# hvasbath/beat

Hardware: AMD Instinct MI355X
Metric: SMC chain-steps/s (FFI seismic gfstacking 400 patches x 64 targets x 4096 samples) (higher is better)
Workload: dtype f64; 1 GPU; BASELINE configs[2]: FFI seismic gfstacking, 400 patches x 64 targets x 4096 samples, library (64,400,3,25,4096) f64 = 62.9 GB in HBM, nearest_neighbor, covariance scalar; population SURVEY 8(d): nucleation U over the 20x20 fault, time 0; chains_per_gpu=512, global_chains=512, parallelism=chains sharded over 1 GPU(s), library replicated

## Files before the change

### beat_amd/csrc/ctx.hpp

```cpp
#pragma once
#include <hip/hip_runtime.h>

#include <cstdarg>
#include <cstdint>
#include <cstdio>
#include <cstring>
#include <map>
#include <memory>
#include <string>
#include <vector>

#include "../../include/beat_amd.h"

struct beatamd_ctx;

namespace beatamd {

void set_error(const char *fmt, ...);

#define BA_HIP(expr)                                                                         \
    do {                                                                                     \
        hipError_t e_ = (expr);                                                              \
        if (e_ != hipSuccess) {                                                              \
            beatamd::set_error("%s:%d: %s -> %s", __FILE__, __LINE__, #expr,                 \
// ... 178 lines not shown
    mutable DevMem<double> pole_coef;
    mutable int64_t pole_chains = 0;
};

struct GeomSources {
    int nsrc = 0;
    DevMem<int32_t> kind;
    DevMem<int64_t> poff;
    DevMem<double> pfix;
    DevMem<double> east, north, los;
    int64_t Nobs = 0;
    double nu = 0.25;
};

struct FfiModel {
    beatamd_ffi_layout layout;
    int32_t nsub = 0;
    std::vector<int32_t> ndip, nstrike, patch_off;
    std::vector<double> patch_size;
    int64_t P = 0;
    DevMem<int32_t> d_ndip, d_nstrike, d_patch_off;
    DevMem<double> d_patch_size;
    std::vector<Wavemap> wavemaps;
    bool has_geo = false;
    Geodetic geo;
    bool geo_is_geometry = false;
    GeomSources geom;
    int32_t lap = -1;
    int64_t nllk() const;
    bool obs_quads_valid = false;
    std::vector<double> obs_quads;
    DevMem<double> d_obs_quads;
    int32_t lsq_var = -1, lsq_zero_var = -1;
    bool lsq_blocks_valid = false;
    DevMem<double> lsq_GG, lsq_LtL;
};

struct HyperModel {
    int64_t nterm = 0, nh = 0;
    DevMem<double> M, slog;
    DevMem<int32_t> kind, hp_index;
    int32_t ngroups = 0, group_end[8] = {0, 0, 0, 0, 0, 0, 0, 0};
};

constexpr int KNOB_UNSET = -2147483647;
#define BEATAMD_GF_KNOBS(X) \
    X(gf_kernel, "BEATAMD_GF_KERNEL") X(gs_cg, "BEATAMD_GS_CG") X(gs_ws, "BEATAMD_GS_WS") X(gs_dma, "BEATAMD_GS_DMA") X(gs_nt, "BEATAMD_GS_NT") \
    X(ws_map, "BEATAMD_WS_MAP") X(gs_pair, "BEATAMD_GS_PAIR") X(gs_nthint, "BEATAMD_GS_NTHINT") X(gs_order, "BEATAMD_GS_ORDER") \
    X(gs_fit, "BEATAMD_GS_FIT") X(gs_win, "BEATAMD_GS_WIN") X(gf_tinv, "BEATAMD_GF_TINV") X(gs_tune, "BEATAMD_GS_TUNE") \
    X(gf_order, "BEATAMD_GF_ORDER") X(gf_cgroup, "BEATAMD_GF_CGROUP") X(gs_ml, "BEATAMD_GS_ML") X(gc_global, "BEATAMD_GC_GLOBAL") \
    X(gc_sort, "BEATAMD_GC_SORT") X(gc_keys, "BEATAMD_GC_KEYS") X(gc_bands, "BEATAMD_GC_BANDS") X(gr_cap, "BEATAMD_GR_CAP") \
    X(gr_pass_alloc, "BEATAMD_GR_PASS_ALLOC") X(gr_var, "BEATAMD_GR_VAR") X(sweep_v1, "BEATAMD_SWEEP_V1") X(qf_band, "BEATAMD_QF_BAND") \
    X(qf_fuse, "BEATAMD_QF_FUSE") X(gf_split, "BEATAMD_GF_SPLIT") X(gm_wave, "BEATAMD_GM_WAVE") X(skip_parked, "BEATAMD_SKIP_PARKED") \
    X(td_strip, "BEATAMD_TD_STRIP")
struct GfKnobs {
#define X(member, env) int member = KNOB_UNSET;
    BEATAMD_GF_KNOBS(X)
#undef X
    void read_env();
    static int get(int v, int dflt) { return v == KNOB_UNSET ? dflt : v; }
    static bool is(int v, int x) { return v != KNOB_UNSET && v == x; }
    static bool set(int v) { return v != KNOB_UNSET; }
};

struct KTimer {
    double total_ms = 0;
    int64_t n = 0;
    std::vector<std::pair<hipEvent_t, hipEvent_t>> pending;
};

}

struct beatamd_ctx {
    int device = 0;
    hipStream_t stream = nullptr, own_stream = nullptr;
    bool timing = false;
    std::map<std::string, beatamd::KTimer> timers;
    std::vector<hipEvent_t> event_pool;
    int *d_status = nullptr;
    std::vector<beatamd::DevBuf> scratch_bufs;
    std::vector<std::unique_ptr<beatamd::SeisStore>> seislibs;
    std::vector<std::unique_ptr<beatamd::GeoLib>> geolibs;
    std::vector<std::unique_ptr<beatamd::GeoEnsemble>> geoens;
    std::vector<std::unique_ptr<beatamd::WeightSet>> wsets;
    std::vector<std::unique_ptr<beatamd::Laplacian>> laps;
    std::vector<std::unique_ptr<beatamd::FfiModel>> models;
    std::vector<std::unique_ptr<beatamd::HyperModel>> hypers;
    int num_cu = 256;
    char last_gf_kernel[96] = "";
    int64_t gs_ngtp = 0, gs_N = 0;
    double gs_trep = 1;
    int gs_nvar = 1;
    bool gs_has_passes = false;
    char gf_plan[384] = "";
    char gf_tune_log[512] = "";
    uint32_t *h_umax = nullptr;
    hipEvent_t umax_event = nullptr;
    bool umax_pending = false;
    int umax_hist = -1, umax_hist_cg = 0;
    std::map<std::vector<int64_t>, std::pair<int, int>> gs_tuned;
    int gs_cg = 0;
    beatamd::GfKnobs knobs;
    bool knobs_live = false;
    uint32_t *step_dev = nullptr;
    std::map<int64_t, beatamd::DevMem<double>> twiddles;

    int get_scratch(int slot, size_t bytes, void **out);
// ... 69 lines not shown
```

### beat_amd/csrc/gfshared.hip

```cpp
#include "kernels.hpp"
#include "misfit.hpp"

namespace beatamd {

constexpr int GS_NT_MAX = 64;
constexpr int GS_NTHINT_DEFAULT = 1;
constexpr int GS_WS_DEFAULT = 1;

struct GroupTabArgs {
    int nrow, nvar, CG;
    int64_t C, T, P, DS;
    const uint32_t *rowoff;
    const double *fac;
    ChainVec slips[4];
    int ucap, ustride;
    uint32_t *urows;
    uint32_t *uent;
    int nissue;
    int windowed;
    int depth;
    uint32_t *ucount;
    uint32_t *umax;
    uint16_t *slot;
    double *w;
// ... 97 lines not shown
                int cost = (tid < 32 && wcnt < a.depth)
                    ? ((__popc(wmask & mm) << 12) | (wcnt << 6) | tid) : 0x7fffffff;
#pragma unroll
                for (int off = 32; off > 0; off >>= 1) cost = min(cost, __shfl_xor(cost, off, 64));
                const int w = cost & 63;
                if (tid == w) {
                    slt[ridx] = (uint32_t)(w + 32 * wcnt);
                    wmask |= mm;
                    wcnt++;
                }
            }
        }
        __syncthreads();
        for (int i = tid; i < total; i += CG) flags[lst[i]] = slt[i];
        __syncthreads();
    }
    {
        const uint32_t last = total > 0 ? a.urows[gtp * a.ustride + total - 1] : (uint32_t)row0;
        for (int i = total + tid; i < a.ustride; i += CG) a.urows[gtp * a.ustride + i] = last;
        const int nw = a.nissue, kstr = a.ustride / nw;
        for (int i = tid; i < a.ustride; i += CG) {
            const uint32_t r = (i < total) ? a.urows[gtp * a.ustride + i] : last;
            uint32_t *e = a.uent + ((gtp * nw + (i % nw)) * kstr + (i / nw)) * 2;
            e[0] = r;
            e[1] = (i < total) ? flags[r - (uint32_t)row0] : 0u;
        }
    }
    for (int k = 0; k < a.nrow; k++)
        a.slot[(gtp * a.nrow + k) * CG + tid] = live ? (uint16_t)flags[v[k]] : (uint16_t)0;
    for (int iv = 0; iv < a.nvar; iv++) {
        double s = 0.0;
        if (live) s = a.slips[iv].base[c * a.slips[iv].stride + a.slips[iv].off + p];
        double *w = a.w + (int64_t)iv * a.w_var_stride;
        if (a.nrow == 1) {
            if (t == 0) w[(g * a.P + p) * CG + tid] = s;
        } else {
            for (int k = 0; k < 4; k++) {
                double f = live ? a.fac[((c * a.T + t) * a.P + p) * 4 + k] : 0.0;
                w[(gtp * 4 + k) * CG + tid] = f * s;
            }
        }
    }
}

struct GsArgs {
    const double *G[4];
    const float *G32[4];
    int f32pair;
    int nvar, nrow;
    int64_t C, T, P, N;
    int CG, ucap, ustride, ntile, nt;
    int dma;
    int ws;
    int nthint;
    int xcd_order;
    int64_t ngroups;
    const int32_t *tslot;
    int64_t Ttab, rows_per_target;
    const uint32_t *guard_umax;
    int guard_mode, guard_fit;
    const uint32_t *nv;
    int64_t vmax;
    const uint32_t *order;
    const uint32_t *urows, *uent, *ucount;
    const uint16_t *slot;
    const double *w;
    int64_t w_var_stride;
    const double *data, *wscalar;
    double *out, *partial;
    const double *band_w;
    double *edges;
};

typedef double v2d __attribute__((ext_vector_type(2)));

template <int OFF>
__device__ __forceinline__ void lds_rd8(v2d (&x)[8], uint32_t addr, int tok)
{
    asm("ds_read_b128 %0, %8 offset:%c10\n\t"
        "ds_read_b128 %1, %8 offset:%c10+16\n\t"
        "ds_read_b128 %2, %8 offset:%c10+32\n\t"
        "ds_read_b128 %3, %8 offset:%c10+48\n\t"
        "ds_read_b128 %4, %8 offset:%c10+64\n\t"
        "ds_read_b128 %5, %8 offset:%c10+80\n\t"
        "ds_read_b128 %6, %8 offset:%c10+96\n\t"
        "ds_read_b128 %7, %8 offset:%c10+112"
        : "=v"(x[0]), "=v"(x[1]), "=v"(x[2]), "=v"(x[3]), "=v"(x[4]), "=v"(x[5]), "=v"(x[6]), "=v"(x[7])
        : "v"(addr), "s"(tok), "n"(OFF));
}

template <int NLEFT>
__device__ __forceinline__ void lds_wait8(v2d (&x)[8])
{
    asm("s_waitcnt lgkmcnt(%c8)"
        : "+v"(x[0]), "+v"(x[1]), "+v"(x[2]), "+v"(x[3]), "+v"(x[4]), "+v"(x[5]), "+v"(x[6]), "+v"(x[7])
        : "n"(NLEFT));
}

template <int OFF>
__device__ __forceinline__ void lds_rd8_b64(double (&x)[8], uint32_t addr, int tok)
{
    asm("ds_read_b64 %0, %8 offset:%c10\n\t"
        "ds_read_b64 %1, %8 offset:%c10+8\n\t"
        "ds_read_b64 %2, %8 offset:%c10+16\n\t"
        "ds_read_b64 %3, %8 offset:%c10+24\n\t"
        "ds_read_b64 %4, %8 offset:%c10+32\n\t"
        "ds_read_b64 %5, %8 offset:%c10+40\n\t"
        "ds_read_b64 %6, %8 offset:%c10+48\n\t"
        "ds_read_b64 %7, %8 offset:%c10+56"
        : "=v"(x[0]), "=v"(x[1]), "=v"(x[2]), "=v"(x[3]), "=v"(x[4]), "=v"(x[5]), "=v"(x[6]), "=v"(x[7])
        : "v"(addr), "s"(tok), "n"(OFF));
}

template <int OFF>
__device__ __forceinline__ void lds_rd8_b32(float (&x)[8], uint32_t addr, int tok)
{
    asm("ds_read_b32 %0, %8 offset:%c10\n\t"
        "ds_read_b32 %1, %8 offset:%c10+4\n\t"
        "ds_read_b32 %2, %8 offset:%c10+8\n\t"
        "ds_read_b32 %3, %8 offset:%c10+12\n\t"
        "ds_read_b32 %4, %8 offset:%c10+16\n\t"
        "ds_read_b32 %5, %8 offset:%c10+20\n\t"
        "ds_read_b32 %6, %8 offset:%c10+24\n\t"
        "ds_read_b32 %7, %8 offset:%c10+28"
        : "=v"(x[0]), "=v"(x[1]), "=v"(x[2]), "=v"(x[3]), "=v"(x[4]), "=v"(x[5]), "=v"(x[6]), "=v"(x[7])
        : "v"(addr), "s"(tok), "n"(OFF));
}

typedef float v2f __attribute__((ext_vector_type(2)));

template <int SCALE, int OFF, typename PAIR>
__device__ __forceinline__ void lds_rd4_pair(PAIR (&x)[4], uint32_t addr, int tok)
{
    if constexpr (SCALE == 1)
        asm("ds_read_b64 %0, %4 offset:%c6\n\t"
            "ds_read_b64 %1, %4 offset:%c6+8\n\t"
            "ds_read_b64 %2, %4 offset:%c6+16\n\t"
            "ds_read_b64 %3, %4 offset:%c6+24"
            : "=v"(x[0]), "=v"(x[1]), "=v"(x[2]), "=v"(x[3])
            : "v"(addr), "s"(tok), "n"(OFF));
    else
        asm("ds_read_b128 %0, %4 offset:%c6\n\t"
            "ds_read_b128 %1, %4 offset:%c6+16\n\t"
            "ds_read_b128 %2, %4 offset:%c6+32\n\t"
            "ds_read_b128 %3, %4 offset:%c6+48"
            : "=v"(x[0]), "=v"(x[1]), "=v"(x[2]), "=v"(x[3])
            : "v"(addr), "s"(tok), "n"(2 * OFF));
}

template <int NLEFT, typename PAIR>
__device__ __forceinline__ void lds_wait4_pair(PAIR (&x)[4])
{
    asm("s_waitcnt lgkmcnt(%c4)" : "+v"(x[0]), "+v"(x[1]), "+v"(x[2]), "+v"(x[3]) : "n"(NLEFT));
}

template <int NLEFT>
__device__ __forceinline__ void lds_wait8_b64(double (&x)[8])
{
    asm("s_waitcnt lgkmcnt(%c8)"
        : "+v"(x[0]), "+v"(x[1]), "+v"(x[2]), "+v"(x[3]), "+v"(x[4]), "+v"(x[5]), "+v"(x[6]), "+v"(x[7])
        : "n"(NLEFT));
}


// ... 449 lines not shown
            for (int gq = 0; gq < NG; gq++) {
                v2f(&cur)[4] = (gq & 1) ? yb : ya;
                if (gq + 1 < NG) lds_wait4_pair<4>(cur); else lds_wait4_pair<0>(cur);
                __builtin_amdgcn_sched_barrier(0);
#pragma unroll
                for (int q = 0; q < 4; q++) {
                    acc[gq * 8 + 2 * q] = fma((double)cur[q].x, w, acc[gq * 8 + 2 * q]);
                    acc[gq * 8 + 2 * q + 1] = fma((double)cur[q].y, w, acc[gq * 8 + 2 * q + 1]);
                }
                __builtin_amdgcn_sched_barrier(0);
                if (gq + 2 < NG) switch (gq + 2) {
                case 2: lds_rd4_pair<1, 64>(cur, xs, s); break;
                case 3: lds_rd4_pair<1, 96>(cur, xs, s); break;
                case 4: lds_rd4_pair<1, 128>(cur, xs, s); break;
                case 5: lds_rd4_pair<1, 160>(cur, xs, s); break;
                case 6: lds_rd4_pair<1, 192>(cur, xs, s); break;
                case 7: lds_rd4_pair<1, 224>(cur, xs, s); break;
                default: break;
                }
                __builtin_amdgcn_sched_barrier(0);
            }
        }
    }
    GS_DMA_FINISH()
}



#define BA_FMA8 \
    "v_fmac_f64 %0, %8, %16\n\tv_fmac_f64 %1, %9, %16\n\tv_fmac_f64 %2, %10, %16\n\tv_fmac_f64 %3, %11, %16\n\t" \
    "v_fmac_f64 %4, %12, %16\n\tv_fmac_f64 %5, %13, %16\n\tv_fmac_f64 %6, %14, %16\n\tv_fmac_f64 %7, %15, %16\n\t"
#define BA_RD8(OFF) \
    "ds_read_b64 %8, %17 offset:" #OFF "\n\tds_read_b64 %9, %17 offset:" #OFF "+8\n\t" \
    "ds_read_b64 %10, %17 offset:" #OFF "+16\n\tds_read_b64 %11, %17 offset:" #OFF "+24\n\t" \
    "ds_read_b64 %12, %17 offset:" #OFF "+32\n\tds_read_b64 %13, %17 offset:" #OFF "+40\n\t" \
    "ds_read_b64 %14, %17 offset:" #OFF "+48\n\tds_read_b64 %15, %17 offset:" #OFF "+56"
#define BA_ACC8(G) \
    "+v"(acc[G * 8]), "+v"(acc[G * 8 + 1]), "+v"(acc[G * 8 + 2]), "+v"(acc[G * 8 + 3]), "+v"(acc[G * 8 + 4]), \
        "+v"(acc[G * 8 + 5]), "+v"(acc[G * 8 + 6]), "+v"(acc[G * 8 + 7])
#define BA_Y8(Y) "+v"(Y[0]), "+v"(Y[1]), "+v"(Y[2]), "+v"(Y[3]), "+v"(Y[4]), "+v"(Y[5]), "+v"(Y[6]), "+v"(Y[7])
#define BA_FMA4A \
    "v_fmac_f64 %0, %8, %16\n\tv_fmac_f64 %1, %9, %16\n\tv_fmac_f64 %2, %10, %16\n\tv_fmac_f64 %3, %11, %16\n\t"
#define BA_FMA4B \
    "v_fmac_f64 %4, %12, %16\n\tv_fmac_f64 %5, %13, %16\n\tv_fmac_f64 %6, %14, %16\n\tv_fmac_f64 %7, %15, %16\n\t"
#define BA_RD4A(OFF) \
    "ds_read_b64 %8, %17 offset:" #OFF "\n\tds_read_b64 %9, %17 offset:" #OFF "+8\n\t" \
    "ds_read_b64 %10, %17 offset:" #OFF "+16\n\tds_read_b64 %11, %17 offset:" #OFF "+24\n\t"
#define BA_RD4B(OFF) \
    "ds_read_b64 %12, %17 offset:" #OFF "+32\n\tds_read_b64 %13, %17 offset:" #OFF "+40\n\t" \
    "ds_read_b64 %14, %17 offset:" #OFF "+48\n\tds_read_b64 %15, %17 offset:" #OFF "+56"
#define BA_GROUP(G, Y, OFFNEXT) \
    asm("s_waitcnt lgkmcnt(12)\n\t" BA_FMA4A BA_RD4A(OFFNEXT) "s_waitcnt lgkmcnt(12)\n\t" BA_FMA4B BA_RD4B(OFFNEXT) \
        : BA_ACC8(G), BA_Y8(Y) : "v"(w), "v"(xs))

template <int NROW, int MODE, int NB, int NTH>
__global__ void __launch_bounds__(768) __attribute__((amdgpu_waves_per_eu(3, 3)))
k_gfstack_ws(GsArgs a)
{
    constexpr int CW = 8, LW = 4;
    constexpr int GS_NT = 64;
    constexpr int GS_PITCH = GS_NT + 1;
    constexpr int KPRE = 16;
    extern __shared__ __attribute__((aligned(16))) double xbuf[];
    constexpr int CG = CW * 64;
    const int tid = threadIdx.x, lane = tid & 63;
    const int wave = __builtin_amdgcn_readfirstlane(tid >> 6);
    GS_BLOCK_DECODE(a, g, t, tile)
    int64_t gt, tbase;
    gs_table_cell(a, g, t, gt, tbase);
    const int64_t N = a.N;
    const int64_t n0 = (int64_t)tile * GS_NT;
    const uint32_t lds0 = (uint32_t)(uintptr_t)(__attribute__((address_space(3))) void *)xbuf;
    const int bufsz = (a.ucap + 1) * GS_PITCH;
    const int P = a.nv ? (int)__builtin_amdgcn_readfirstlane((int)a.nv[gt]) : (int)a.P;
    const int nvar = a.nvar;
    const int nsteps = P * nvar;

    if (wave >= CW) {
        GS_LOADER_PROGRAM(0, 8, double, G_a = a.G[iv] + tbase)
        return;
    }

    static_assert(NROW == 1, "the loader / consumer kernel exists for single-row interpolation");
    const int64_t c = a.order ? (int64_t)a.order[g * CG + tid] : g * CG + tid;
    for (int i = tid; i < NB * GS_PITCH; i += CG) xbuf[(i / GS_PITCH) * bufsz + a.ucap * GS_PITCH + (i % GS_PITCH)] = 0.0;
    __builtin_amdgcn_fence(__ATOMIC_RELEASE, "workgroup");
    double acc[GS_NT];
#pragma unroll
    for (int i = 0; i < GS_NT; i++) acc[i] = 0.0;
    uint32_t sl_n;
    double wl_n;
    const uint32_t voff_s = (uint32_t)tid * 2u;
    const char *const slot_base = reinterpret_cast<const char *>(a.slot + (gt * a.vmax) * CG);
    const char *const w_base = reinterpret_cast<const char *>(a.w + (gt * a.vmax) * CG);
    const uint32_t slot_step = (uint32_t)(CG * 2);
    const uint32_t w_step = (uint32_t)(CG * 8);
    const int64_t w_var_bytes = a.w_var_stride * 8;
    auto tab_slot = [&](int p) { return slot_base + (uint32_t)p * slot_step; };
    auto tab_w = [&](int p, int iv) {
        return w_base + (uint32_t)p * w_step + (nvar == 1 ? (int64_t)0 : (int64_t)iv * w_var_bytes);
    };
    auto fetch_tabs = [&](const char *ps, const char *pw) {
        asm("global_load_ushort %0, %1, %2" : "=v"(sl_n) : "v"(voff_s), "s"(ps));
        uint32_t voff_w;
        asm("v_lshlrev_b32 %1, 2, %2\n\t"
            "global_load_dwordx2 %0, %1, %3" : "=v"(wl_n), "=&v"(voff_w) : "v"(voff_s), "s"(pw));
    };
    auto row_address = [&](uint32_t base) {
        uint32_t x;
        asm("s_waitcnt vmcnt(0)\n\t"
            "v_lshl_add_u32 %0, %1, 6, %1\n\t"
            "v_lshl_add_u32 %0, %0, 3, %2" : "=&v"(x) : "v"(sl_n), "s"(base), "v"(wl_n));
        return x;
    };
    auto landed_weight = [&](uint32_t after) {
        double x;
        asm("v_mov_b64 %0, %1" : "=v"(x) : "v"(wl_n), "v"(after));
        return x;
    };
    static_assert(GS_PITCH == 65, "row_address multiplies by 65");
    constexpr int NG8 = GS_NT / 8;
    static_assert(NG8 == 8, "the read schedule below is written for 64-sample tiles");
    double ya[8], yb[8];
    int p1 = 0, iv1 = 0;
    gs_advance(p1, iv1, P, nvar);
    int gbuf = 0;
    const int ring = NB * bufsz;
    double w;
    uint32_t xs;
    if (__ballot(c < a.C) == 0) {
        for (int s = 0; s <= nsteps; s++) __builtin_amdgcn_s_barrier();
    } else {
    fetch_tabs(tab_slot(0), tab_w(0, 0));
    xs = row_address(lds0);
    w = landed_weight(xs);
    __builtin_amdgcn_sched_barrier(0);
    __builtin_amdgcn_s_barrier();
    __builtin_amdgcn_sched_barrier(0);
    lds_rd8_b64<0>(ya, xs, -1);
    lds_rd8_b64<64>(yb, xs, -1);
    __builtin_amdgcn_sched_barrier(0);
    fetch_tabs(tab_slot(p1), tab_w(p1, iv1));
    gs_advance(p1, iv1, P, nvar);
    const char *ps_run = tab_slot(p1), *pw_run = tab_w(p1, iv1);
    int iv_run = iv1;
    const int64_t dw_next = (nvar == 1) ? (int64_t)w_step : w_var_bytes;
    const int64_t dw_wrap = (int64_t)w_step - (int64_t)(nvar - 1) * w_var_bytes;
#pragma clang loop unroll(disable)
    for (int s = 0; s < nsteps; s++) {
        int gnext = gbuf + bufsz;
        if (gnext == ring) gnext = 0;
        __builtin_amdgcn_sched_barrier(0);
        BA_GROUP(0, ya, 128);
        BA_GROUP(1, yb, 192);
        BA_GROUP(2, ya, 256);
        BA_GROUP(3, yb, 320);
        BA_GROUP(4, ya, 384);
        BA_GROUP(5, yb, 448);
        __builtin_amdgcn_sched_barrier(0);
        asm("s_waitcnt lgkmcnt(0)\n\t" BA_FMA8
            : BA_ACC8(6), BA_Y8(ya) : "v"(w), "v"(xs), "v"(yb[0]), "v"(yb[1]), "v"(yb[2]), "v"(yb[3]),
              "v"(yb[4]), "v"(yb[5]), "v"(yb[6]), "v"(yb[7]));
        __builtin_amdgcn_sched_barrier(0);
        gbuf = gnext;
        const uint32_t xs_n = row_address(lds0 + (uint32_t)(gbuf * 8));
        __builtin_amdgcn_sched_barrier(0);
        __builtin_amdgcn_s_barrier();
        __builtin_amdgcn_sched_barrier(0);
        lds_rd8_b64<0>(ya, xs_n, s);
        __builtin_amdgcn_sched_barrier(0);
        asm(BA_FMA8
            "v_mov_b64 %16, %18\n\t" BA_RD8(64)
            : BA_ACC8(7), BA_Y8(yb), "+v"(w) : "v"(xs_n), "v"(wl_n));
        xs = xs_n;
        __builtin_amdgcn_sched_barrier(0);
        fetch_tabs(ps_run, pw_run);
        {
            uint32_t ds;
            int64_t dw;
            asm("s_add_i32 %0, %0, 1\n\t"
                "s_cmp_eq_u32 %0, %3\n\t"
                "s_cselect_b32 %0, 0, %0\n\t"
                "s_cselect_b32 %1, %4, 0\n\t"
                "s_cselect_b64 %2, %5, %6"
                : "+s"(iv_run), "=&s"(ds), "=&s"(dw) : "s"(nvar), "s"(slot_step), "s"(dw_wrap), "s"(dw_next) : "scc");
            ps_run += ds;
            pw_run += dw;
        }
    }
    asm volatile("s_waitcnt vmcnt(0) lgkmcnt(0)"
                 : "+v"(ya[0]), "+v"(ya[1]), "+v"(ya[2]), "+v"(ya[3]), "+v"(ya[4]), "+v"(ya[5]), "+v"(ya[6]),
                   "+v"(ya[7]), "+v"(yb[0]), "+v"(yb[1]), "+v"(yb[2]), "+v"(yb[3]), "+v"(yb[4]), "+v"(yb[5]),
                   "+v"(yb[6]), "+v"(yb[7]), "+v"(sl_n), "+v"(wl_n));
    __builtin_amdgcn_sched_barrier(0);
    }

    const bool live = (c < a.C);
    const int nvalid = (int)min((int64_t)GS_NT, N - n0);
    if (MODE == GF_STORE_SYN) {
        if (live) {
            gs_store_syn<GS_NT>(a.out + (c * a.T + t) * N + n0, acc, nvalid);
        }
        return;
    }
    __builtin_amdgcn_s_barrier();
    if (tid < GS_NT) xbuf[tid] = (tid < nvalid) ? a.data[t * N + n0 + tid] : 0.0;
    if (MODE == GF_RESID_BAND1 && tid >= GS_NT && tid < 3 * GS_NT)
        xbuf[tid] = ((tid - GS_NT) >> 1) < nvalid ? a.band_w[(t * N + n0) * 2 + (tid - GS_NT)] : 0.0;
    __builtin_amdgcn_fence(__ATOMIC_RELEASE, "workgroup");
    __builtin_amdgcn_s_barrier();
    __builtin_amdgcn_fence(__ATOMIC_ACQUIRE, "workgroup");
    if (MODE == GF_RESID_BAND1) {
        const double *wbt = xbuf + GS_NT;
        const auto resid = [&](int i) { return xbuf[i] - acc[i]; };
        const double rfirst = resid(0);
        const Band1Tile tl = band1_tile<true, GS_NT>(resid, [&](int i, int b) { return wbt[2 * i + b]; }, nvalid, n0 + nvalid == N);
        if (live) {
            const int64_t e = (c * a.T + t) * a.ntile + tile;
            a.partial[e] = tl.q;
            a.edges[2 * e] = rfirst;
            a.edges[2 * e + 1] = tl.r_last;
        }
    } else if (MODE == GF_RESID_STORE) {
        constexpr int TP = 17;
        double *tw = xbuf + GS_NT + wave * (64 * TP);
        const uint32_t cu = (uint32_t)min(c, (int64_t)0xffffffff);
        const int sl = lane & 15;
#pragma unroll
        for (int i0 = 0; i0 < GS_NT; i0 += 16) {
#pragma unroll
            for (int i = 0; i < 16; i++) tw[lane * TP + i] = xbuf[i0 + i] - acc[i0 + i];
            __builtin_amdgcn_fence(__ATOMIC_RELEASE, "wavefront");
            __builtin_amdgcn_wave_barrier();
            __builtin_amdgcn_fence(__ATOMIC_ACQUIRE, "wavefront");
#pragma unroll
            for (int k = 0; k < 16; k++) {
                const double v = tw[(k * 4 + (lane >> 4)) * TP + sl];
                const int64_t cc = (int64_t)(uint32_t)__shfl((int)cu, k * 4 + (lane >> 4));
                if (cc < a.C && i0 + sl < nvalid) a.out[(cc * a.T + t) * N + n0 + i0 + sl] = v;
            }
            __builtin_amdgcn_fence(__ATOMIC_RELEASE, "wavefront");
            __builtin_amdgcn_wave_barrier();
        }
    } else {
        const double q = gs_misfit_scalar<GS_NT>(a.wscalar[t], acc, xbuf, nvalid);
        if (live) a.partial[(c * a.T + t) * a.ntile + tile] = q;
    }
}


#undef BA_GROUP
#undef BA_RD4B
#undef BA_RD4A
#undef BA_FMA4B
#undef BA_FMA4A
#undef BA_Y8
#undef BA_ACC8
#undef BA_RD8
#undef BA_FMA8

template <int F32, int MODE, int NB, int NTH>
__global__ void __launch_bounds__(768) __attribute__((amdgpu_waves_per_eu(3, 3)))
k_gfstack_wsp(GsArgs a)
{
    constexpr int CW = 8, LW = 4;
    constexpr int GS_NT = 64;
    constexpr int GS_PITCH = GS_NT + 2;
    constexpr int ES = F32 ? 4 : 8;
    typedef typename std::conditional<F32 != 0, float, double>::type elem_t;
    typedef typename std::conditional<F32 != 0, v2f, v2d>::type pair_t;
    constexpr int KPRE = 16;
    extern __shared__ __attribute__((aligned(16))) double xbuf[];
    constexpr int CG = CW * 64;
    const int tid = threadIdx.x, lane = tid & 63;
    const int wave = __builtin_amdgcn_readfirstlane(tid >> 6);
    GS_BLOCK_DECODE(a, g, t, tile)
    int64_t gt, tbase;
    gs_table_cell(a, g, t, gt, tbase);
    const int64_t N = a.N;
    const int64_t n0 = (int64_t)tile * GS_NT;
    const uint32_t lds0 = (uint32_t)(uintptr_t)(__attribute__((address_space(3))) void *)xbuf;
    const int bufsz = (a.ucap + 1) * GS_PITCH;
    const int P = a.nv ? (int)__builtin_amdgcn_readfirstlane((int)a.nv[gt]) : (int)a.P;
    const int nvar = a.nvar;
    const int nsteps = P * nvar;

    if (wave >= CW) {
        GS_LOADER_PROGRAM(F32, ES, elem_t, if constexpr (F32 != 0) G_a = a.G32[iv] + tbase; else G_a = a.G[iv] + tbase)
        return;
    }

    const int64_t c = a.order ? (int64_t)a.order[g * CG + tid] : g * CG + tid;
    for (int i = tid; i < NB * GS_PITCH; i += CG)
        reinterpret_cast<elem_t *>(xbuf)[(i / GS_PITCH) * bufsz + a.ucap * GS_PITCH + (i % GS_PITCH)] = (elem_t)0;
    __builtin_amdgcn_fence(__ATOMIC_RELEASE, "workgroup");
    double acc[GS_NT];
#pragma unroll
    for (int i = 0; i < GS_NT; i++) acc[i] = 0.0;
    uint32_t sl_n;
    double wl_n;
    const uint32_t voff_s = (uint32_t)tid * 2u;
    const char *const slot_base = reinterpret_cast<const char *>(a.slot + (gt * a.vmax) * CG);
    const char *const w_base = reinterpret_cast<const char *>(a.w + (gt * a.vmax) * CG);
// ... 522 lines not shown
    const int mode = g.mode;
    const int64_t ngroups = (k.C + WS_CG - 1) / WS_CG;
    const int64_t GT = ngroups * Ttab, GTP = GT * L.P;
    const int64_t bound = std::min<int64_t>(WS_CG, L.D * L.S);
    const int cap = bound <= 32 ? 32 : bound <= 64 ? 64 : WS_CAP_MAX;
    const int maxpass = (int)((bound + cap - 1) / cap);
    const int64_t vmax = L.P * maxpass;

    WsTabArgs ta;
    memset(&ta, 0, sizeof(ta));
    ta.nvar = k.nvar; ta.cap = cap;
    ta.C = k.C; ta.T = Ttab; ta.P = L.P; ta.DS = L.D * L.S; ta.vmax = vmax;
    ta.rowoff = ln.rowoff;
    for (int v = 0; v < k.nvar; v++) ta.slips[v] = k.slips[v];
    ta.R = p.R;
    if (ngroups > 1 && k.order_key[0].base && k.order_key[1].base && GfKnobs::get(kn.gc_global, 1) != 0)
        BA_TRY(launch_chain_members(ctx, k.C, k.order_key, WS_CG, ngroups, &ta.order, GfKnobs::get(kn.gc_global, 1) == 2));
    BA_TRY(ctx->scratch(SL_GS_UCOUNT, (size_t)(3 * GTP + GT), &ta.utotal));
    ta.npass = ta.utotal + GTP;
    uint32_t *voff = ta.npass + GTP, *nv = voff + GTP;
    const size_t nvs = (size_t)GT * vmax + 3;
    BA_TRY(ctx->scratch(SL_GS_UROWS, nvs, &ta.ucount));
    BA_TRY(ctx->scratch(SL_GS_USLOT, nvs * WS_USTRIDE * 2, &ta.uent));
    BA_TRY(ctx->scratch(SL_GS_SLOT, nvs * WS_CG, &ta.slot));
    ta.w_var_stride = (int64_t)GT * vmax * WS_CG;
    BA_TRY(ctx->scratch(SL_GS_W, (size_t)ta.w_var_stride * k.nvar + (size_t)3 * WS_CG, &ta.w));
    {
        ScopedTimer tm(ctx, "grouptables");
        if (k.active) {
            uint32_t *packed;
            BA_TRY(ctx->scratch(SL_WS_PACK, (size_t)ngroups * WS_CG, &packed));
            hipLaunchKernelGGL(k_ws_pack, dim3((unsigned)ngroups), dim3(WS_CG), 0, ctx->stream, ta.order, k.active, k.C, packed);
            ta.order = packed;
        }
        const bool map = ta.DS <= WS_MAP_MAX && !GfKnobs::is(kn.ws_map, 0);
        const size_t mlds = map ? (size_t)ta.DS * sizeof(uint16_t) : 0;
        if (maxpass > 1) {
            if (map) hipLaunchKernelGGL((k_ws_tables<0, 1>), dim3((unsigned)GTP), dim3(WS_CG), mlds, ctx->stream, ta);
            else hipLaunchKernelGGL((k_ws_tables<0, 0>), dim3((unsigned)GTP), dim3(WS_CG), 0, ctx->stream, ta);
            hipLaunchKernelGGL(k_ws_scan, dim3((unsigned)GT), dim3(256), 0, ctx->stream, ta.npass, voff, nv, L.P);
            ta.voff = voff;
        }
        if (map) hipLaunchKernelGGL((k_ws_tables<1, 1>), dim3((unsigned)GTP), dim3(WS_CG), mlds, ctx->stream, ta);
        else hipLaunchKernelGGL((k_ws_tables<1, 0>), dim3((unsigned)GTP), dim3(WS_CG), 0, ctx->stream, ta);
    }
    BA_HIP(hipGetLastError());

    GsArgs a;
    const bool f32 = p.f32, pair64 = p.pair64;
    gs_common_args(a, k, p, ln, ngroups);
    a.nrow = 1;
    a.CG = WS_CG; a.ucap = cap; a.ustride = WS_USTRIDE;
    a.nt = 64; a.dma = 2; a.ws = 3;
    a.ntile = (int)((L.N + 63) / 64);
    a.nv = maxpass > 1 ? nv : nullptr;
    a.vmax = vmax;
    a.order = ta.order;
    a.uent = ta.uent; a.ucount = ta.ucount; a.slot = ta.slot; a.w = ta.w;
    a.w_var_stride = ta.w_var_stride;
    if (mode == GF_RESID_SCALAR || mode == GF_RESID_BAND1) BA_TRY(ctx->scratch(SL_PARTIAL, (size_t)k.C * L.T * a.ntile, &a.partial));
    if (mode == GF_RESID_BAND1) {
        BA_TRY(ctx->scratch(SL_EDGES, (size_t)k.C * L.T * a.ntile * 2, &a.edges));
        a.band_w = k.band_w;
    }
    const int64_t nblocks = gs_grid(a, kn);
    BA_CHECK(nblocks < (int64_t)0x7fffffff, BEATAMD_EINVAL, "gfstack: batch too large");
    size_t lds = f32 ? (size_t)(cap + 1) * (64 + 2) * sizeof(float) * 3
                     : (size_t)(cap + 1) * (64 + (pair64 ? 2 : 1)) * sizeof(double) * 3;
    lds = std::max<size_t>(lds, (64 + 8 * 64 * 17) * sizeof(double));
    BA_CHECK(lds <= 160 * 1024, BEATAMD_EINVAL, "internal: k_gfstack_ws row buffers exceed LDS");
    if (f32 || pair64)
        snprintf(ctx->last_gf_kernel, sizeof(ctx->last_gf_kernel), "k_gfstack_ws%s<%d,%d,%d>", f32 ? "32" : "p64", mode, a.ws,
                 a.nthint);
    else
        snprintf(ctx->last_gf_kernel, sizeof(ctx->last_gf_kernel), "k_gfstack_ws<%d,%d,%d,%d>", 1, mode, a.ws, a.nthint);
    snprintf(ctx->gf_plan, sizeof(ctx->gf_plan),
             "loader/consumer kernel: 512-chain groups, nearest neighbour; %d row slots per LDS buffer (a patch can touch min(512, "
             "D*S = %lld) rows), %s", cap, (long long)(L.D * L.S),
             maxpass > 1 ? "patches that touch more are staged in passes of equal size" : "one pass per patch");
    gs_record_stats(ctx, k, GTP, Ttab, WS_CG, maxpass > 1);
    {
        ScopedTimer tm(ctx, "gfstack");
        BA_TRY(launch_ws(mode, dim3((unsigned)nblocks), lds, ctx->stream, a, f32 ? 1 : (pair64 ? 2 : 0)));
    }
    BA_HIP(hipGetLastError());
    if (a.partial)
        BA_TRY(launch_sum_tiles(ctx, a.partial, k.C * L.T, a.ntile, k.quad, nullptr, 0, a.edges, k.band_w, L.T, L.N));
    return BEATAMD_OK;
}

static int launch_dma_twin(beatamd_ctx *ctx, const GfStackCall &k, const GfPlan &p, const GfGroup &g, GsArgs &shared, int twin,
                           int ucap, bool windowed, int64_t GTP)
{
    const SeisLib &L = *k.libs[0];
    const int nrow = p.nrow, CG = g.cg, mode = g.mode;
    GsArgs a = shared;
    a.ucap = ucap;
    a.guard_mode = twin;
    size_t lds = (size_t)ucap * (a.nt + 2) * sizeof(double);
    BA_CHECK(2 * lds <= 158 * 1024, BEATAMD_EINVAL, "internal: k_gfstack_dma row buffers exceed LDS");
    a.dma = GfKnobs::is(p.knobs->gs_dma, 1) ? 1 : 2;
    if (a.nt == 32 && a.dma != 2) { a.nt = 64; a.ntile = (int)((L.N + 63) / 64); lds = (size_t)ucap * (a.nt + 2) * sizeof(double); }
    BA_CHECK(CG != 1024 || a.dma == 2, BEATAMD_EINVAL, "gfstack: 1024-chain groups need the LDS-DMA kernel");
    BA_CHECK(!windowed || a.dma == 2, BEATAMD_EINVAL, "internal: window slots need the ds_read_b64 kernel");
    a.ws = 0;
    a.f32pair = 0;
// ... 116 lines not shown
```

Baseline: 94360 chain-steps/s.

## Split sample accumulation across 2 or 4 lanes per chain in sparse tail waves

In the warp-specialized gfstack kernel, a wave whose live chains form a contiguous prefix of at most 32 (or 16) lanes now gives each chain 2 (or 4) lanes. Each lane accumulates a strided subset of the 64 samples, and the partial results are transposed back through LDS before the shared epilogue. This spreads the LDS reads and FMAs of underfilled tail waves across otherwise idle lanes. The cost is more code, extra register pressure and an extra LDS transpose, and the path is controlled by a new ws_tail knob that defaults to on.

New measurement: 94260 chain-steps/s. No clear change (-0.1%).

```diff
diff --git a/beat_amd/csrc/ctx.hpp b/beat_amd/csrc/ctx.hpp
--- a/beat_amd/csrc/ctx.hpp
+++ b/beat_amd/csrc/ctx.hpp
@@ -254,7 +254,7 @@
     X(gc_sort, "BEATAMD_GC_SORT") X(gc_keys, "BEATAMD_GC_KEYS") X(gc_bands, "BEATAMD_GC_BANDS") X(gr_cap, "BEATAMD_GR_CAP") \
     X(gr_pass_alloc, "BEATAMD_GR_PASS_ALLOC") X(gr_var, "BEATAMD_GR_VAR") X(sweep_v1, "BEATAMD_SWEEP_V1") X(qf_band, "BEATAMD_QF_BAND") \
     X(qf_fuse, "BEATAMD_QF_FUSE") X(gf_split, "BEATAMD_GF_SPLIT") X(gm_wave, "BEATAMD_GM_WAVE") X(skip_parked, "BEATAMD_SKIP_PARKED") \
-    X(td_strip, "BEATAMD_TD_STRIP")
+    X(td_strip, "BEATAMD_TD_STRIP") X(ws_tail, "BEATAMD_WS_TAIL")
 struct GfKnobs {
 #define X(member, env) int member = KNOB_UNSET;
     BEATAMD_GF_KNOBS(X)
diff --git a/beat_amd/csrc/gfshared.hip b/beat_amd/csrc/gfshared.hip
--- a/beat_amd/csrc/gfshared.hip
+++ b/beat_amd/csrc/gfshared.hip
@@ -173,6 +173,7 @@
     int CG, ucap, ustride, ntile, nt;
     int dma;
     int ws;
+    int tail;
     int nthint;
     int xcd_order;
     int64_t ngroups;
@@ -231,6 +232,21 @@
         "ds_read_b64 %7, %8 offset:%c10+56"
         : "=v"(x[0]), "=v"(x[1]), "=v"(x[2]), "=v"(x[3]), "=v"(x[4]), "=v"(x[5]), "=v"(x[6]), "=v"(x[7])
         : "v"(addr), "s"(tok), "n"(OFF));
+}
+
+template <int OFF, int ST>
+__device__ __forceinline__ void lds_rd8_b64s(double (&x)[8], uint32_t addr, int tok)
+{
+    asm("ds_read_b64 %0, %8 offset:%c10\n\t"
+        "ds_read_b64 %1, %8 offset:%c10+%c11\n\t"
+        "ds_read_b64 %2, %8 offset:%c10+2*%c11\n\t"
+        "ds_read_b64 %3, %8 offset:%c10+3*%c11\n\t"
+        "ds_read_b64 %4, %8 offset:%c10+4*%c11\n\t"
+        "ds_read_b64 %5, %8 offset:%c10+5*%c11\n\t"
+        "ds_read_b64 %6, %8 offset:%c10+6*%c11\n\t"
+        "ds_read_b64 %7, %8 offset:%c10+7*%c11"
+        : "=v"(x[0]), "=v"(x[1]), "=v"(x[2]), "=v"(x[3]), "=v"(x[4]), "=v"(x[5]), "=v"(x[6]), "=v"(x[7])
+        : "v"(addr), "s"(tok), "n"(OFF), "n"(ST));
 }
 
 template <int OFF>
@@ -786,6 +802,38 @@
 #define BA_GROUP(G, Y, OFFNEXT) \
     asm("s_waitcnt lgkmcnt(12)\n\t" BA_FMA4A BA_RD4A(OFFNEXT) "s_waitcnt lgkmcnt(12)\n\t" BA_FMA4B BA_RD4B(OFFNEXT) \
         : BA_ACC8(G), BA_Y8(Y) : "v"(w), "v"(xs))
+#define BA_TACC8(G) \
+    "+v"(ta[G * 8]), "+v"(ta[G * 8 + 1]), "+v"(ta[G * 8 + 2]), "+v"(ta[G * 8 + 3]), "+v"(ta[G * 8 + 4]), \
+        "+v"(ta[G * 8 + 5]), "+v"(ta[G * 8 + 6]), "+v"(ta[G * 8 + 7])
+#define BA_RD4AS(OFF, ST) \
+    "ds_read_b64 %8, %17 offset:" #OFF "\n\tds_read_b64 %9, %17 offset:" #OFF "+" #ST "\n\t" \
+    "ds_read_b64 %10, %17 offset:" #OFF "+2*" #ST "\n\tds_read_b64 %11, %17 offset:" #OFF "+3*" #ST "\n\t"
+#define BA_RD4BS(OFF, ST) \
+    "ds_read_b64 %12, %17 offset:" #OFF "+4*" #ST "\n\tds_read_b64 %13, %17 offset:" #OFF "+5*" #ST "\n\t" \
+    "ds_read_b64 %14, %17 offset:" #OFF "+6*" #ST "\n\tds_read_b64 %15, %17 offset:" #OFF "+7*" #ST
+#define BA_TGROUP(G, Y, OFFNEXT, ST) \
+    asm("s_waitcnt lgkmcnt(12)\n\t" BA_FMA4A BA_RD4AS(OFFNEXT, ST) "s_waitcnt lgkmcnt(12)\n\t" BA_FMA4B BA_RD4BS(OFFNEXT, ST) \
+        : BA_TACC8(G), BA_Y8(Y) : "v"(w), "v"(xs))
+#define BA_TGROUP_LAST_READS(G, Y, Y2) \
+    asm("s_waitcnt lgkmcnt(0)\n\t" BA_FMA8 \
+        : BA_TACC8(G), BA_Y8(Y) : "v"(w), "v"(xs), "v"(Y2[0]), "v"(Y2[1]), "v"(Y2[2]), "v"(Y2[3]), \
+          "v"(Y2[4]), "v"(Y2[5]), "v"(Y2[6]), "v"(Y2[7]))
+#define BA_TGROUP_NEXT(G, Y, OFF1, ST) \
+    asm(BA_FMA8 "v_mov_b64 %16, %18\n\t" BA_RD4AS(OFF1, ST) BA_RD4BS(OFF1, ST) \
+        : BA_TACC8(G), BA_Y8(Y), "+v"(w) : "v"(xs_n), "v"(wl_n))
+#define BA_TAB_ADVANCE() \
+    { \
+        uint32_t ds; \
+        int64_t dw; \
+        asm("s_add_i32 %0, %0, 1\n\t" \
+            "s_cmp_eq_u32 %0, %3\n\t" \
+            "s_cselect_b32 %0, 0, %0\n\t" \
+            "s_cselect_b32 %1, %4, 0\n\t" \
+            "s_cselect_b64 %2, %5, %6" \
+            : "+s"(iv_run), "=&s"(ds), "=&s"(dw) : "s"(nvar), "s"(slot_step), "s"(dw_wrap), "s"(dw_next) : "scc"); \
+        ps_run += ds; \
+        pw_run += dw; \
+    }
 
 template <int NROW, int MODE, int NB, int NTH>
 __global__ void __launch_bounds__(768) __attribute__((amdgpu_waves_per_eu(3, 3)))
@@ -817,6 +865,12 @@
 
     static_assert(NROW == 1, "the loader / consumer kernel exists for single-row interpolation");
     const int64_t c = a.order ? (int64_t)a.order[g * CG + tid] : g * CG + tid;
+    const uint64_t live_mask = __ballot(c < a.C);
+    int mt = 1;
+    if (a.tail && (live_mask & (live_mask + 1)) == 0) {
+        const int k = __popcll(live_mask);
+        mt = k <= 16 ? 4 : (k <= 32 ? 2 : 1);
+    }
     for (int i = tid; i < NB * GS_PITCH; i += CG) xbuf[(i / GS_PITCH) * bufsz + a.ucap * GS_PITCH + (i % GS_PITCH)] = 0.0;
     __builtin_amdgcn_fence(__ATOMIC_RELEASE, "workgroup");
     double acc[GS_NT];
@@ -834,12 +888,13 @@
     auto tab_w = [&](int p, int iv) {
         return w_base + (uint32_t)p * w_step + (nvar == 1 ? (int64_t)0 : (int64_t)iv * w_var_bytes);
     };
-    auto fetch_tabs = [&](const char *ps, const char *pw) {
-        asm("global_load_ushort %0, %1, %2" : "=v"(sl_n) : "v"(voff_s), "s"(ps));
+    auto fetch_tabs_at = [&](uint32_t voff, const char *ps, const char *pw) {
+        asm("global_load_ushort %0, %1, %2" : "=v"(sl_n) : "v"(voff), "s"(ps));
         uint32_t voff_w;
         asm("v_lshlrev_b32 %1, 2, %2\n\t"
-            "global_load_dwordx2 %0, %1, %3" : "=v"(wl_n), "=&v"(voff_w) : "v"(voff_s), "s"(pw));
+            "global_load_dwordx2 %0, %1, %3" : "=v"(wl_n), "=&v"(voff_w) : "v"(voff), "s"(pw));
     };
+    auto fetch_tabs = [&](const char *ps, const char *pw) { fetch_tabs_at(voff_s, ps, pw); };
     auto row_address = [&](uint32_t base) {
         uint32_t x;
         asm("s_waitcnt vmcnt(0)\n\t"
@@ -862,8 +917,140 @@
     const int ring = NB * bufsz;
     double w;
     uint32_t xs;
-    if (__ballot(c < a.C) == 0) {
+    auto epilogue = [&]() {
+        const bool live = (c < a.C);
+        const int nvalid = (int)min((int64_t)GS_NT, N - n0);
+        if (MODE == GF_STORE_SYN) {
+            if (live) {
+                gs_store_syn<GS_NT>(a.out + (c * a.T + t) * N + n0, acc, nvalid);
+            }
+            return;
+        }
+        __builtin_amdgcn_s_barrier();
+        if (tid < GS_NT) xbuf[tid] = (tid < nvalid) ? a.data[t * N + n0 + tid] : 0.0;
+        if (MODE == GF_RESID_BAND1 && tid >= GS_NT && tid < 3 * GS_NT)
+            xbuf[tid] = ((tid - GS_NT) >> 1) < nvalid ? a.band_w[(t * N + n0) * 2 + (tid - GS_NT)] : 0.0;
+        __builtin_amdgcn_fence(__ATOMIC_RELEASE, "workgroup");
+        __builtin_amdgcn_s_barrier();
+        __builtin_amdgcn_fence(__ATOMIC_ACQUIRE, "workgroup");
+        if (MODE == GF_RESID_BAND1) {
+            const double *wbt = xbuf + GS_NT;
+            const auto resid = [&](int i) { return xbuf[i] - acc[i]; };
+            const double rfirst = resid(0);
+            const Band1Tile tl = band1_tile<true, GS_NT>(resid, [&](int i, int b) { return wbt[2 * i + b]; }, nvalid, n0 + nvalid == N);
+            if (live) {
+                const int64_t e = (c * a.T + t) * a.ntile + tile;
+                a.partial[e] = tl.q;
+                a.edges[2 * e] = rfirst;
+                a.edges[2 * e + 1] = tl.r_last;
+            }
+        } else if (MODE == GF_RESID_STORE) {
+            constexpr int TP = 17;
+            double *tw = xbuf + GS_NT + wave * (64 * TP);
+            const uint32_t cu = (uint32_t)min(c, (int64_t)0xffffffff);
+            const int sl = lane & 15;
+#pragma unroll
+            for (int i0 = 0; i0 < GS_NT; i0 += 16) {
+#pragma unroll
+                for (int i = 0; i < 16; i++) tw[lane * TP + i] = xbuf[i0 + i] - acc[i0 + i];
+                __builtin_amdgcn_fence(__ATOMIC_RELEASE, "wavefront");
+                __builtin_amdgcn_wave_barrier();
+                __builtin_amdgcn_fence(__ATOMIC_ACQUIRE, "wavefront");
+#pragma unroll
+                for (int k = 0; k < 16; k++) {
+                    const double v = tw[(k * 4 + (lane >> 4)) * TP + sl];
+                    const int64_t cc = (int64_t)(uint32_t)__shfl((int)cu, k * 4 + (lane >> 4));
+                    if (cc < a.C && i0 + sl < nvalid) a.out[(cc * a.T + t) * N + n0 + i0 + sl] = v;
+                }
+                __builtin_amdgcn_fence(__ATOMIC_RELEASE, "wavefront");
+                __builtin_amdgcn_wave_barrier();
+            }
+        } else {
+            const double q = gs_misfit_scalar<GS_NT>(a.wscalar[t], acc, xbuf, nvalid);
+            if (live) a.partial[(c * a.T + t) * a.ntile + tile] = q;
+        }
+    };
+    auto gather_tail = [&](auto mc) {
+        constexpr int M = decltype(mc)::value;
+        static_assert(M == 2 || M == 4, "2 or 4 lanes per chain");
+        constexpr int ST = 8 * M;
+        constexpr int NA = GS_NT / M;
+        double ta[NA];
+#pragma unroll
+        for (int i = 0; i < NA; i++) ta[i] = 0.0;
+        const int q = lane & (M - 1), pl = lane / M;
+        const uint32_t qoff = (uint32_t)q * 8u;
+        const uint32_t voff_t = (uint32_t)(tid - lane + pl) * 2u;
+        fetch_tabs_at(voff_t, tab_slot(0), tab_w(0, 0));
+        xs = row_address(lds0) + qoff;
+        w = landed_weight(xs);
+        __builtin_amdgcn_sched_barrier(0);
+        __builtin_amdgcn_s_barrier();
+        __builtin_amdgcn_sched_barrier(0);
+        lds_rd8_b64s<0, ST>(ya, xs, -1);
+        lds_rd8_b64s<8 * ST, ST>(yb, xs, -1);
+        __builtin_amdgcn_sched_barrier(0);
+        fetch_tabs_at(voff_t, tab_slot(p1), tab_w(p1, iv1));
+        gs_advance(p1, iv1, P, nvar);
+        const char *ps_run = tab_slot(p1), *pw_run = tab_w(p1, iv1);
+        int iv_run = iv1;
+        const int64_t dw_next = (nvar == 1) ? (int64_t)w_step : w_var_bytes;
+        const int64_t dw_wrap = (int64_t)w_step - (int64_t)(nvar - 1) * w_var_bytes;
+#pragma clang loop unroll(disable)
+        for (int s = 0; s < nsteps; s++) {
+            int gnext = gbuf + bufsz;
+            if (gnext == ring) gnext = 0;
+            __builtin_amdgcn_sched_barrier(0);
+            if constexpr (M == 2) {
+                BA_TGROUP(0, ya, 256, 16);
+                BA_TGROUP(1, yb, 384, 16);
+                __builtin_amdgcn_sched_barrier(0);
+                BA_TGROUP_LAST_READS(2, ya, yb);
+            } else {
+                BA_TGROUP_LAST_READS(0, ya, yb);
+            }
+            __builtin_amdgcn_sched_barrier(0);
+            gbuf = gnext;
+            const uint32_t xs_n = row_address(lds0 + (uint32_t)(gbuf * 8)) + qoff;
+            __builtin_amdgcn_sched_barrier(0);
+            __builtin_amdgcn_s_barrier();
+            __builtin_amdgcn_sched_barrier(0);
+            lds_rd8_b64s<0, ST>(ya, xs_n, s);
+            __builtin_amdgcn_sched_barrier(0);
+            if constexpr (M == 2) BA_TGROUP_NEXT(3, yb, 128, 16);
+            else BA_TGROUP_NEXT(1, yb, 256, 32);
+            xs = xs_n;
+            __builtin_amdgcn_sched_barrier(0);
+            fetch_tabs_at(voff_t, ps_run, pw_run);
+            BA_TAB_ADVANCE()
+        }
+        asm volatile("s_waitcnt vmcnt(0) lgkmcnt(0)"
+                     : "+v"(ya[0]), "+v"(ya[1]), "+v"(ya[2]), "+v"(ya[3]), "+v"(ya[4]), "+v"(ya[5]), "+v"(ya[6]),
+                       "+v"(ya[7]), "+v"(yb[0]), "+v"(yb[1]), "+v"(yb[2]), "+v"(yb[3]), "+v"(yb[4]), "+v"(yb[5]),
+                       "+v"(yb[6]), "+v"(yb[7]), "+v"(sl_n), "+v"(wl_n));
+        __builtin_amdgcn_sched_barrier(0);
+        constexpr int TP = 33, TH = GS_NT / 2;
+        double *tt = xbuf + 3 * GS_NT + wave * (32 * TP);
+#pragma unroll
+        for (int h = 0; h < 2; h++) {
+#pragma unroll
+            for (int i = 0; i < TH / M; i++) tt[pl * TP + M * i + q] = ta[h * (TH / M) + i];
+            __builtin_amdgcn_fence(__ATOMIC_RELEASE, "wavefront");
+            __builtin_amdgcn_wave_barrier();
+            __builtin_amdgcn_fence(__ATOMIC_ACQUIRE, "wavefront");
+#pragma unroll
+            for (int i = 0; i < TH; i++) acc[h * TH + i] = tt[(lane & 31) * TP + i];
+            __builtin_amdgcn_fence(__ATOMIC_RELEASE, "wavefront");
+            __builtin_amdgcn_wave_barrier();
+        }
+    };
+    if (live_mask == 0) {
         for (int s = 0; s <= nsteps; s++) __builtin_amdgcn_s_barrier();
+    } else if (mt != 1) {
+        if (mt == 4) gather_tail(std::integral_constant<int, 4>());
+        else gather_tail(std::integral_constant<int, 2>());
+        epilogue();
+        return;
     } else {
     fetch_tabs(tab_slot(0), tab_w(0, 0));
     xs = row_address(lds0);
@@ -909,18 +1096,7 @@
         xs = xs_n;
         __builtin_amdgcn_sched_barrier(0);
         fetch_tabs(ps_run, pw_run);
-        {
-            uint32_t ds;
-            int64_t dw;
-            asm("s_add_i32 %0, %0, 1\n\t"
-                "s_cmp_eq_u32 %0, %3\n\t"
-                "s_cselect_b32 %0, 0, %0\n\t"
-                "s_cselect_b32 %1, %4, 0\n\t"
-                "s_cselect_b64 %2, %5, %6"
-                : "+s"(iv_run), "=&s"(ds), "=&s"(dw) : "s"(nvar), "s"(slot_step), "s"(dw_wrap), "s"(dw_next) : "scc");
-            ps_run += ds;
-            pw_run += dw;
-        }
+        BA_TAB_ADVANCE()
     }
     asm volatile("s_waitcnt vmcnt(0) lgkmcnt(0)"
                  : "+v"(ya[0]), "+v"(ya[1]), "+v"(ya[2]), "+v"(ya[3]), "+v"(ya[4]), "+v"(ya[5]), "+v"(ya[6]),
@@ -929,60 +1105,17 @@
     __builtin_amdgcn_sched_barrier(0);
     }
 
-    const bool live = (c < a.C);
-    const int nvalid = (int)min((int64_t)GS_NT, N - n0);
-    if (MODE == GF_STORE_SYN) {
-        if (live) {
-            gs_store_syn<GS_NT>(a.out + (c * a.T + t) * N + n0, acc, nvalid);
-        }
-        return;
-    }
-    __builtin_amdgcn_s_barrier();
-    if (tid < GS_NT) xbuf[tid] = (tid < nvalid) ? a.data[t * N + n0 + tid] : 0.0;
-    if (MODE == GF_RESID_BAND1 && tid >= GS_NT && tid < 3 * GS_NT)
-        xbuf[tid] = ((tid - GS_NT) >> 1) < nvalid ? a.band_w[(t * N + n0) * 2 + (tid - GS_NT)] : 0.0;
-    __builtin_amdgcn_fence(__ATOMIC_RELEASE, "workgroup");
-    __builtin_amdgcn_s_barrier();
-    __builtin_amdgcn_fence(__ATOMIC_ACQUIRE, "workgroup");
-    if (MODE == GF_RESID_BAND1) {
-        const double *wbt = xbuf + GS_NT;
-        const auto resid = [&](int i) { return xbuf[i] - acc[i]; };
-        const double rfirst = resid(0);
-        const Band1Tile tl = band1_tile<true, GS_NT>(resid, [&](int i, int b) { return wbt[2 * i + b]; }, nvalid, n0 + nvalid == N);
-        if (live) {
-            const int64_t e = (c * a.T + t) * a.ntile + tile;
-            a.partial[e] = tl.q;
-            a.edges[2 * e] = rfirst;
-            a.edges[2 * e + 1] = tl.r_last;
-        }
-    } else if (MODE == GF_RESID_STORE) {
-        constexpr int TP = 17;
-        double *tw = xbuf + GS_NT + wave * (64 * TP);
-        const uint32_t cu = (uint32_t)min(c, (int64_t)0xffffffff);
-        const int sl = lane & 15;
-#pragma unroll
-        for (int i0 = 0; i0 < GS_NT; i0 += 16) {
-#pragma unroll
-            for (int i = 0; i < 16; i++) tw[lane * TP + i] = xbuf[i0 + i] - acc[i0 + i];
-            __builtin_amdgcn_fence(__ATOMIC_RELEASE, "wavefront");
-            __builtin_amdgcn_wave_barrier();
-            __builtin_amdgcn_fence(__ATOMIC_ACQUIRE, "wavefront");
-#pragma unroll
-            for (int k = 0; k < 16; k++) {
-                const double v = tw[(k * 4 + (lane >> 4)) * TP + sl];
-                const int64_t cc = (int64_t)(uint32_t)__shfl((int)cu, k * 4 + (lane >> 4));
-                if (cc < a.C && i0 + sl < nvalid) a.out[(cc * a.T + t) * N + n0 + i0 + sl] = v;
-            }
-            __builtin_amdgcn_fence(__ATOMIC_RELEASE, "wavefront");
-            __builtin_amdgcn_wave_barrier();
-        }
-    } else {
-        const double q = gs_misfit_scalar<GS_NT>(a.wscalar[t], acc, xbuf, nvalid);
-        if (live) a.partial[(c * a.T + t) * a.ntile + tile] = q;
-    }
-}
-
-
+    epilogue();
+}
+
+
+#undef BA_TAB_ADVANCE
+#undef BA_TGROUP_NEXT
+#undef BA_TGROUP_LAST_READS
+#undef BA_TGROUP
+#undef BA_RD4BS
+#undef BA_RD4AS
+#undef BA_TACC8
 #undef BA_GROUP
 #undef BA_RD4B
 #undef BA_RD4A
@@ -1611,6 +1744,7 @@
     a.nrow = 1;
     a.CG = WS_CG; a.ucap = cap; a.ustride = WS_USTRIDE;
     a.nt = 64; a.dma = 2; a.ws = 3;
+    a.tail = GfKnobs::get(kn.ws_tail, 1) != 0;
     a.ntile = (int)((L.N + 63) / 64);
     a.nv = maxpass > 1 ? nv : nullptr;
     a.vmax = vmax;
```
